# InterlinkLabs/e2e-tts

Hardware: AMD Instinct MI355X
Metric: audio samples/sec (22.05 kHz, batch-32 per GPU, FastSpeech2 + HiFi-GAN inference, ids on host -> int16 PCM on host) (higher is better)
Workload: dtype f32; 1 GPU; B=32/GPU fixed-length L=128 phonemes x 6 frames = T=768 frames (196608 samples, 8.92 s) per utterance; default model_config (6+6 FFT blocks H=384, HiFi-GAN V1), random-init weights; ids of tests/golden/bench_b32.npz (reference-pinned); global_batch=32, parallelism=utterance-sharded x1

## Files before the change

### e2e_tts_amd/csrc/attention.hip

```cpp
#include <math.h>

#include <algorithm>

#include "kernels.h"
#include "tuning.h"

namespace e2etts {

typedef float f32x16 __attribute__((ext_vector_type(16)));
typedef float f32x4v __attribute__((ext_vector_type(4)));
typedef unsigned u32x4v __attribute__((ext_vector_type(4)));

namespace {

__device__ __forceinline__ void lds_barrier() { asm volatile("s_waitcnt lgkmcnt(0)\n\ts_barrier" ::: "memory"); }

__device__ __forceinline__ void wave_lds_fence() {
  __builtin_amdgcn_fence(__ATOMIC_RELEASE, "wavefront");
  __builtin_amdgcn_wave_barrier();
  __builtin_amdgcn_fence(__ATOMIC_ACQUIRE, "wavefront");
}

constexpr int ATT_SEG_CHUNKS = 8;
__device__ __forceinline__ void seg_merge_ml(float& m, float& l, const float m_s, const float l_s, float& a, float& b) {
// ... 98 lines not shown
  }
}

template <int DT>
__device__ __forceinline__ void att_segment_close(f32x16 (&o)[DT], float& m_run, float& l_run, f32x16 (&ot)[DT], float& m_tot, float& l_tot,
                                                  const bool first) {
  if (first) {
#pragma unroll
    for (int d = 0; d < DT; ++d)
#pragma unroll
      for (int r = 0; r < 16; ++r) ot[d][r] = o[d][r];
    m_tot = m_run;
    l_tot = l_run;
  } else {
    float ma, mb;
    seg_merge_ml(m_tot, l_tot, m_run, l_run, ma, mb);
#pragma unroll
    for (int d = 0; d < DT; ++d)
#pragma unroll
      for (int r = 0; r < 16; ++r) ot[d][r] = seg_merge_o(ot[d][r], o[d][r], ma, mb);
  }
  att_clear(o);
  m_run = -INFINITY;
  l_run = 0.f;
}

template <int DT, int DK_BOUND>
__device__ __forceinline__ void att_store_rows(const f32x16 (&o)[DT], const float l, const bool valid, float* __restrict__ orow, const int lh) {
  const float inv = valid ? 1.0f / l : 0.f;
#pragma unroll
  for (int d = 0; d < DT; ++d)
#pragma unroll
    for (int g = 0; g < 4; ++g) {
      if (DK_BOUND % 32 == 0 || d * 32 + 8 * g + 4 * lh < DK_BOUND) {
        float4 v;
        v.x = valid ? o[d][4 * g + 0] * inv : 0.f;
        v.y = valid ? o[d][4 * g + 1] * inv : 0.f;
        v.z = valid ? o[d][4 * g + 2] * inv : 0.f;
        v.w = valid ? o[d][4 * g + 3] * inv : 0.f;
        *reinterpret_cast<float4*>(orow + d * 32 + 8 * g) = v;
      }
    }
}

template <int DK>
__global__ __launch_bounds__(256, 2) void attention_kernel(const float* __restrict__ qkv, float* __restrict__ out,
                                                        const int32_t* __restrict__ lens, int N, int H, float temperature, const RowMap rm) {
  constexpr int LDS_LD = DK + 4;
  constexpr int DT = DK / 32;
  constexpr int QQ = DK / 8;
  constexpr bool HALVES = DT % 2 == 0;
  __shared__ __attribute__((aligned(16))) float Ks[32 * LDS_LD];
  __shared__ __attribute__((aligned(16))) float Vs[32 * LDS_LD];

  const int tid = threadIdx.x, lane = tid & 63, wave = tid >> 6;
  const int li = lane & 31, lh = lane >> 5;
  ATT_BLOCK_OF_GRID(128)
  const int q0 = qblk * 128 + wave * 32;
  const int len = min(lens ? lens[b] : N, N);
  if (qblk * 128 >= len) {
    att_zero_tile<128, 256, DK>(out, b, qblk, head, N, H, tid);
    return;
  }
  const int ld = 3 * H;
  const float* base = qkv + (long long)b * N * ld;
  const float* qp = base + head * DK;
  const float* kp = base + H + head * DK;
  const float* vp = base + 2 * H + head * DK;

  float4 qf[QQ];
  att_load_q_f32(qf, qp + (long long)min(q0 + li, N - 1) * ld + lh * 4);

  f32x16 o[DT];
  att_clear(o);
  float m_run = -INFINITY, l_run = 0.f;
  f32x16 ot[DT];
  att_clear(ot);
  float m_tot = -INFINITY, l_tot = 0.f;

  const int nchunks = (len + 31) / 32;
  for (int sg0 = 0; sg0 < nchunks; sg0 += ATT_SEG_CHUNKS) {
  const int sg1 = min(nchunks, sg0 + ATT_SEG_CHUNKS);
  for (int kc = sg0; kc < sg1; ++kc) {
    __syncthreads();
    for (int i = tid; i < 32 * (DK / 4); i += 256) {
      const int r = i / (DK / 4), c = (i % (DK / 4)) * 4;
      const int key = kc * 32 + r;
      float4 kv = make_float4(0.f, 0.f, 0.f, 0.f), vv = kv;
      if (key < N) {
        kv = *reinterpret_cast<const float4*>(kp + (long long)key * ld + c);
        vv = *reinterpret_cast<const float4*>(vp + (long long)key * ld + c);
      }
      *reinterpret_cast<float4*>(Ks + r * LDS_LD + c) = kv;
      *reinterpret_cast<float4*>(Vs + r * LDS_LD + c) = vv;
    }
    __syncthreads();

    f32x16 s;
#pragma unroll
    for (int r = 0; r < 16; ++r) s[r] = 0.f;
    const float* ka = Ks + li * LDS_LD + lh * 4;
    if constexpr (HALVES) {
      f32x16 s1;
#pragma unroll
      for (int r = 0; r < 16; ++r) s1[r] = 0.f;
      att_qk_f32<0, QQ / 2>(s, ka, qf);
      att_qk_f32<QQ / 2, QQ>(s1, ka, qf);
#pragma unroll
      for (int r = 0; r < 16; ++r) s[r] = s[r] + s1[r];
    } else {
      att_qk_f32<0, QQ>(s, ka, qf);
    }
    float mx = -INFINITY;
#pragma unroll
    for (int r = 0; r < 16; ++r) {
      const int key = kc * 32 + (r & 3) + 8 * (r >> 2) + 4 * lh;
      float v = s[r] / temperature;
      v = key < len ? v : -INFINITY;
      s[r] = v;
      mx = fmaxf(mx, v);
    }
    mx = fmaxf(mx, __shfl_xor(mx, 32));
    const float m_new = fmaxf(m_run, mx);
    const float corr = expf(m_run - m_new);
    float psum = 0.f;
#pragma unroll
    for (int r = 0; r < 16; ++r) {
      const float pv = expf(s[r] - m_new);
      s[r] = pv;
      psum += pv;
    }
    psum += __shfl_xor(psum, 32);
    l_run = l_run * corr + psum;
    m_run = m_new;
    att_pv_f32<DT, LDS_LD>(o, s, corr, Vs + li, lh);
  }
    att_segment_close(o, m_run, l_run, ot, m_tot, l_tot, sg0 == 0);
  }

  const int q = q0 + li;
  if (q < N) att_store_rows<DT, DK>(ot, l_tot, q < len, out + ((long long)b * N + q) * H + head * DK + 4 * lh, lh);
}

template <int DK, int QT>
__global__ __launch_bounds__(QT * 128, 2) void attention_split_kernel(const float* __restrict__ qkv, float* __restrict__ out,
                                                                 const int32_t* __restrict__ lens, int N, int H, float temperature, const RowMap rm,
                                                                 float* __restrict__ ws_o, float* __restrict__ ws_ml, const int par_nseg) {
  constexpr int LDS_LD = DK + 4;
  constexpr int DH = DK / 2;
  constexpr int DTH = DH / 32;
  constexpr int QQH = DH / 8;
  static_assert(DK % 64 == 0, "the split form needs an even number of 32-wide head-dim tiles");
  constexpr int NF4 = 32 * (DK / 4);
  constexpr int NTH = QT * 128;
  constexpr int NLD = (NF4 + NTH - 1) / NTH;
  __shared__ __attribute__((aligned(16))) float Ks[32 * LDS_LD];
  __shared__ __attribute__((aligned(16))) float Vs[32 * LDS_LD];
  __shared__ __attribute__((aligned(16))) float Sx[QT * 2][16 * 64];

  const int tid = threadIdx.x, lane = tid & 63, wave = __builtin_amdgcn_readfirstlane(tid >> 6);
  const int li = lane & 31, lh = lane >> 5;
  const int qt = wave >> 1, part = wave & 1;
  ATT_BLOCK_OF_GRID(QT * 32)
  int seg_id = 0;
  if (par_nseg > 0) {
    seg_id = qblk % par_nseg;
    qblk /= par_nseg;
  }
  const int q0 = qblk * (QT * 32) + qt * 32;
  const int len = min(lens ? lens[b] : N, N);
  if (par_nseg > 0 && qblk * (QT * 32) >= len) return;
  if (qblk * (QT * 32) >= len) {
    att_zero_tile<QT * 32, NTH, DK>(out, b, qblk, head, N, H, tid);
    return;
  }
  const int ld = 3 * H;
  const float* base = qkv + (long long)b * N * ld;
  const float* qp = base + head * DK + part * DH;
  const float* kp = base + H + head * DK;
  const float* vp = base + 2 * H + head * DK;

  float4 qf[QQH];
  att_load_q_f32(qf, qp + (long long)min(q0 + li, N - 1) * ld + lh * 4);
  f32x16 o[DTH];
  att_clear(o);
  float m_run = -INFINITY, l_run = 0.f;

  float4 kreg[NLD], vreg[NLD];
  auto fetch = [&](int kc) __attribute__((always_inline)) {
#pragma unroll
    for (int i = 0; i < NLD; ++i) {
      const int idx = min(tid + i * NTH, NF4 - 1);
      const int r = idx / (DK / 4), c = (idx % (DK / 4)) * 4;
      const int key = min(kc * 32 + r, N - 1);
      kreg[i] = *reinterpret_cast<const float4*>(kp + (long long)key * ld + c);
      vreg[i] = *reinterpret_cast<const float4*>(vp + (long long)key * ld + c);
    }
  };
  auto stash = [&](int kc) __attribute__((always_inline)) {
#pragma unroll
    for (int i = 0; i < NLD; ++i) {
      const int idx = tid + i * NTH;
      if (idx < NF4) {
        const int r = idx / (DK / 4), c = (idx % (DK / 4)) * 4;
        const bool ok = kc * 32 + r < N;
        const float4 kv = make_float4(ok ? kreg[i].x : 0.f, ok ? kreg[i].y : 0.f, ok ? kreg[i].z : 0.f, ok ? kreg[i].w : 0.f);
        const float4 vv = make_float4(ok ? vreg[i].x : 0.f, ok ? vreg[i].y : 0.f, ok ? vreg[i].z : 0.f, ok ? vreg[i].w : 0.f);
        *reinterpret_cast<float4*>(Ks + r * LDS_LD + c) = kv;
        *reinterpret_cast<float4*>(Vs + r * LDS_LD + c) = vv;
      }
    }
  };

  const int nchunks = (len + 31) / 32;
  const int kc_begin = par_nseg > 0 ? seg_id * ATT_SEG_CHUNKS : 0;
  const int kc_end = par_nseg > 0 ? min(nchunks, (seg_id + 1) * ATT_SEG_CHUNKS) : nchunks;
  if (kc_begin >= kc_end) return;
  f32x16 ot[DTH];
  att_clear(ot);
  float m_tot = -INFINITY, l_tot = 0.f;
  fetch(kc_begin);
  for (int sg0 = kc_begin; sg0 < kc_end; sg0 += ATT_SEG_CHUNKS) {
  const int sg1 = min(kc_end, sg0 + ATT_SEG_CHUNKS);
  for (int kc = sg0; kc < sg1; ++kc) {
    lds_barrier();
    stash(kc);
    lds_barrier();
    if (kc + 1 < kc_end) fetch(kc + 1);

    f32x16 s;
#pragma unroll
    for (int r = 0; r < 16; ++r) s[r] = 0.f;
    att_qk_f32<0, QQH>(s, Ks + li * LDS_LD + part * DH + lh * 4, qf);
#pragma unroll
    for (int r = 0; r < 16; ++r) Sx[wave][r * 64 + lane] = s[r];
    lds_barrier();
    {
      const float* s0 = Sx[wave & ~1];
      const float* s1 = Sx[wave | 1];
#pragma unroll
      for (int r = 0; r < 16; ++r) s[r] = s0[r * 64 + lane] + s1[r * 64 + lane];
    }
    const float corr = att_softmax_step<true>(s, kc * 32, lh, len, temperature, m_run, l_run);
    att_pv_f32<DTH, LDS_LD>(o, s, corr, Vs + part * DH + li, lh);
  }
    if (par_nseg == 0) att_segment_close(o, m_run, l_run, ot, m_tot, l_tot, sg0 == kc_begin);
  }

  const int q = q0 + li;
  if (par_nseg > 0) {
    if (q < N) {
      const long long row = (((long long)b * (H / DK) + head) * par_nseg + seg_id) * N + q;
      float* orow = ws_o + row * DK + part * DH + 4 * lh;
#pragma unroll
      for (int d = 0; d < DTH; ++d)
#pragma unroll
        for (int g = 0; g < 4; ++g)
          *reinterpret_cast<float4*>(orow + d * 32 + 8 * g) = make_float4(o[d][4 * g], o[d][4 * g + 1], o[d][4 * g + 2], o[d][4 * g + 3]);
      if (part == 0 && lh == 0) *reinterpret_cast<float2*>(ws_ml + row * 2) = make_float2(m_run, l_run);
    }
    return;
  }
#pragma unroll
  for (int d = 0; d < DTH; ++d)
#pragma unroll
    for (int r = 0; r < 16; ++r) o[d][r] = ot[d][r];
  l_run = l_tot;
  if (q < N) att_store_rows<DTH, DH>(o, l_run, q < len, out + ((long long)b * N + q) * H + head * DK + part * DH + 4 * lh, lh);
}

__global__ void attention_combine_kernel(const float* __restrict__ ws_o, const float* __restrict__ ws_ml, float* __restrict__ out,
                                         const int32_t* __restrict__ lens, int N, int H, int DK, int par_nseg, long long total4) {
  const long long i = (long long)blockIdx.x * blockDim.x + threadIdx.x;
  if (i >= total4) return;
  const int d4 = DK / 4, nh = H / DK;
  const int c4 = (int)(i % d4);
  const int head = (int)((i / d4) % nh);
  const long long bq = i / ((long long)d4 * nh);
  const int q = (int)(bq % N), b = (int)(bq / N);
  const int len = min(lens ? lens[b] : N, N);
  float4 o = make_float4(0.f, 0.f, 0.f, 0.f);
  if (q < len) {
    const int nseg = ((len + 31) / 32 + ATT_SEG_CHUNKS - 1) / ATT_SEG_CHUNKS;
    float m = -INFINITY, l = 0.f;
    for (int sg = 0; sg < nseg; ++sg) {
      const long long row = (((long long)b * nh + head) * par_nseg + sg) * N + q;
      const float2 ml = *reinterpret_cast<const float2*>(ws_ml + row * 2);
      const float4 os = *reinterpret_cast<const float4*>(ws_o + row * DK + c4 * 4);
      if (sg == 0) {
        m = ml.x; l = ml.y; o = os;
      } else {
        float ma, mb;
        seg_merge_ml(m, l, ml.x, ml.y, ma, mb);
        o.x = seg_merge_o(o.x, os.x, ma, mb); o.y = seg_merge_o(o.y, os.y, ma, mb);
        o.z = seg_merge_o(o.z, os.z, ma, mb); o.w = seg_merge_o(o.w, os.w, ma, mb);
      }
    }
    const float inv = 1.0f / l;
    o.x *= inv; o.y *= inv; o.z *= inv; o.w *= inv;
  }
  *reinterpret_cast<float4*>(out + ((long long)b * N + q) * H + head * DK + c4 * 4) = o;
}

template <int DK>
__global__ __launch_bounds__(256, 2) void rel_attention_kernel(const float* __restrict__ qkv, const float* __restrict__ pos, int pos_rows,
                                                               const float* __restrict__ ub, const float* __restrict__ vb,
                                                               float* __restrict__ out, int N, int H, float temperature) {
  static_assert(DK % 8 == 0, "head dim must be a multiple of 8");
  constexpr int DT = (DK + 31) / 32;
  constexpr int LDS_LD = DT * 32 + 4;
  constexpr int QQ = DK / 8;
  constexpr int GLD = 68;
  constexpr int NPRE = QQ;
  __shared__ __attribute__((aligned(16))) float Ks[32 * LDS_LD];
  __shared__ __attribute__((aligned(16))) float Vs[32 * LDS_LD];
  __shared__ __attribute__((aligned(16))) float Gt[4][32 * GLD];

  const int tid = threadIdx.x, lane = tid & 63, wave = __builtin_amdgcn_readfirstlane(tid >> 6);
  const int li = lane & 31, lh = lane >> 5;
  const int b = blockIdx.z, head = blockIdx.y;
  const int i0 = blockIdx.x * 128 + wave * 32;
  const int ld = 3 * H;
  const float* base = qkv + (long long)b * N * ld;
  const float* qp = base + head * DK;
  const float* kp = base + H + head * DK;
  const float* vp = base + 2 * H + head * DK;
  const float* ph = pos + (long long)head * pos_rows * DK;
  float* const gt = Gt[wave];

  const int qi = min(i0 + li, N - 1);
  float4 qf[QQ], qx[QQ];
  auto load_qx = [&](const int row) __attribute__((always_inline)) {
    const float* qr = qp + (row * ld + lh * 4);
    const float* vr = vb + head * DK + lh * 4;
#pragma unroll
    for (int qq = 0; qq < QQ; ++qq) {
      const float4 a = *reinterpret_cast<const float4*>(qr + qq * 8), v4 = *reinterpret_cast<const float4*>(vr + qq * 8);
      qx[qq] = make_float4(a.x + v4.x, a.y + v4.y, a.z + v4.z, a.w + v4.w);
    }
  };
  {
    const float* qr = qp + (qi * ld + lh * 4);
    const float* ur = ub + head * DK + lh * 4;
#pragma unroll
    for (int qq = 0; qq < QQ; ++qq) {
      const float4 a = *reinterpret_cast<const float4*>(qr + qq * 8), u4 = *reinterpret_cast<const float4*>(ur + qq * 8);
      qf[qq] = make_float4(a.x + u4.x, a.y + u4.y, a.z + u4.z, a.w + u4.w);
    }
  }
  load_qx(qi);
  if (DK % 32) {
    for (int i = tid; i < 32 * (DT * 32 - DK); i += 256) {
      const int r = i / (DT * 32 - DK), c = DK + i % (DT * 32 - DK);
      Vs[r * LDS_LD + c] = 0.f;
    }
  }

  f32x16 o[DT];
  att_clear(o);
  float m_run = -INFINITY, l_run = 0.f;

  typedef f32x4v PRE_T;
  auto band_fetch = [&](PRE_T (&pre)[NPRE], const int row_start) __attribute__((always_inline)) {
    const int row = min(max(row_start + li, 0), pos_rows - 1);
    const float* pr = ph + (row * DK + lh * 4);
#pragma unroll
    for (int qq = 0; qq < QQ; ++qq) pre[qq] = *reinterpret_cast<const f32x4v*>(pr + qq * 8);
  };
  auto band_tile = [&](const PRE_T (&pre)[NPRE], const float4 (&x)[QQ]) __attribute__((always_inline)) -> f32x16 {
    f32x16 g;
#pragma unroll
    for (int r = 0; r < 16; ++r) g[r] = 0.f;
#pragma unroll
    for (int qq = 0; qq < QQ; ++qq) {
      g = __builtin_amdgcn_mfma_f32_32x32x2f32(pre[qq].x, x[qq].x, g, 0, 0, 0);
      g = __builtin_amdgcn_mfma_f32_32x32x2f32(pre[qq].y, x[qq].y, g, 0, 0, 0);
      g = __builtin_amdgcn_mfma_f32_32x32x2f32(pre[qq].z, x[qq].z, g, 0, 0, 0);
      g = __builtin_amdgcn_mfma_f32_32x32x2f32(pre[qq].w, x[qq].w, g, 0, 0, 0);
    }
    return g;
  };
  auto skew = [&](const f32x16& g0, const f32x16& g1, float (&term)[16], const bool diag) __attribute__((always_inline)) {
    wave_lds_fence();
#pragma unroll
    for (int q4 = 0; q4 < 4; ++q4) {
      const int t = 8 * q4 + 4 * lh;
      *reinterpret_cast<float4*>(gt + li * GLD + t) = make_float4(g0[4 * q4], g0[4 * q4 + 1], g0[4 * q4 + 2], g0[4 * q4 + 3]);
      *reinterpret_cast<float4*>(gt + li * GLD + 32 + t) = make_float4(g1[4 * q4], g1[4 * q4 + 1], g1[4 * q4 + 2], g1[4 * q4 + 3]);
    }
    wave_lds_fence();
#pragma unroll
    for (int r = 0; r < 16; ++r) {
      const int c = (r & 3) + 8 * (r >> 2) + 4 * lh;
      const float v = gt[li * GLD + (c - li + 31)];
      const bool keep = diag && c <= li, zero = diag && c == li + 1;
      term[r] = keep ? term[r] : (zero ? 0.f : v);
    }
  };
  auto new_tile_row = [&](const int j0, const bool upper) { return upper ? j0 - i0 - 1 : N + j0 - i0; };
  PRE_T pre[NPRE];
  f32x16 ghi;
#pragma unroll
  for (int r = 0; r < 16; ++r) ghi[r] = 0.f;

  const int nchunks = (N + 31) / 32;
  for (int kc = 0; kc < nchunks; ++kc) {
    const int j0 = kc * 32;
    __syncthreads();
    for (int i = tid; i < 32 * (DK / 4); i += 256) {
      const int r = i / (DK / 4), c = (i % (DK / 4)) * 4;
      const int key = j0 + r;
      float4 kv = make_float4(0.f, 0.f, 0.f, 0.f), vv = kv;
      if (key < N) {
        kv = *reinterpret_cast<const float4*>(kp + (key * ld + c));
        vv = *reinterpret_cast<const float4*>(vp + (key * ld + c));
      }
      *reinterpret_cast<float4*>(Ks + r * LDS_LD + c) = kv;
      *reinterpret_cast<float4*>(Vs + r * LDS_LD + c) = vv;
    }
    float pterm[16];
    if (j0 <= i0) {
      if (kc == 0) {
        band_fetch(pre, new_tile_row(j0, false) - 32);
        ghi = band_tile(pre, qx);
        band_fetch(pre, new_tile_row(j0, false));
      }
      const f32x16 g1 = band_tile(pre, qx);
      if (j0 < i0) band_fetch(pre, new_tile_row(j0 + 32, false));
      skew(ghi, g1, pterm, false);
      ghi = g1;
    }
    if (j0 >= i0) {
      if (j0 == i0) {
        load_qx(min(qi + 1, N - 1));
        band_fetch(pre, new_tile_row(j0, true) - 32);
        ghi = band_tile(pre, qx);
        band_fetch(pre, new_tile_row(j0, true));
      }
      const f32x16 g1 = band_tile(pre, qx);
      if (kc + 1 < nchunks) band_fetch(pre, new_tile_row(j0 + 32, true));
      skew(ghi, g1, pterm, j0 == i0);
      ghi = g1;
      if (j0 == i0 + 32 && li == 31 && lh == 0) pterm[0] = 0.f;
    }
    __syncthreads();

    f32x16 s;
#pragma unroll
    for (int r = 0; r < 16; ++r) s[r] = pterm[r];
    att_qk_f32<0, QQ>(s, Ks + li * LDS_LD + lh * 4, qf);
    const float corr = att_softmax_step<true>(s, j0, lh, N, temperature, m_run, l_run);
    att_pv_f32<DT, LDS_LD>(o, s, corr, Vs + li, lh);
  }

  const int q = i0 + li;
  if (q < N) att_store_rows<DT, DK>(o, l_run, true, out + ((long long)b * N + q) * H + head * DK + 4 * lh, lh);
}

typedef __bf16 bf16x8_t __attribute__((ext_vector_type(8)));
typedef __bf16 bf16x2_t __attribute__((ext_vector_type(2)));

__device__ __forceinline__ unsigned pk_bf16(float a, float b) {
  const bf16x2_t r = {(__bf16)a, (__bf16)b};
  return __builtin_bit_cast(unsigned, r);
}
__device__ __forceinline__ void split8(const float* v, bf16x8_t& hi, bf16x8_t& lo) {
  uint4 h, l;
  unsigned* hp = reinterpret_cast<unsigned*>(&h);
  unsigned* lp = reinterpret_cast<unsigned*>(&l);
#pragma unroll
  for (int i = 0; i < 4; ++i) {
    hp[i] = pk_bf16(v[2 * i], v[2 * i + 1]);
    const float h0 = __builtin_bit_cast(float, hp[i] << 16), h1 = __builtin_bit_cast(float, hp[i] & 0xffff0000u);
    lp[i] = pk_bf16(v[2 * i] - h0, v[2 * i + 1] - h1);
  }
  hi = __builtin_bit_cast(bf16x8_t, h);
  lo = __builtin_bit_cast(bf16x8_t, l);
}

constexpr int VS = 36;

template <int NS>
__device__ __forceinline__ void att_load_q_x3(bf16x8_t (&qh)[NS], bf16x8_t (&ql)[NS], const float* __restrict__ qr) {
#pragma unroll
  for (int s = 0; s < NS; ++s) {
    const float4 a = *reinterpret_cast<const float4*>(qr + s * 16), c = *reinterpret_cast<const float4*>(qr + s * 16 + 4);
    const float v[8] = {a.x, a.y, a.z, a.w, c.x, c.y, c.z, c.w};
    split8(v, qh[s], ql[s]);
  }
}

template <int DK, int VROWS>
__device__ __forceinline__ void att_stage_kv_x3(unsigned* Kh, unsigned* Vt, const int r, const int c4, const float4 kv, const float4 vv) {
  constexpr int KS = DK + 4;
  const unsigned k0 = pk_bf16(kv.x, kv.y), k1 = pk_bf16(kv.z, kv.w);
  const float kx = __builtin_bit_cast(float, k0 << 16), ky = __builtin_bit_cast(float, k0 & 0xffff0000u);
  const float kz = __builtin_bit_cast(float, k1 << 16), kw = __builtin_bit_cast(float, k1 & 0xffff0000u);
  *reinterpret_cast<uint2*>(Kh + r * KS + c4 * 2) = make_uint2(k0, k1);
  *reinterpret_cast<uint2*>(Kh + r * KS + DK / 2 + c4 * 2) = make_uint2(pk_bf16(kv.x - kx, kv.y - ky), pk_bf16(kv.z - kz, kv.w - kw));
  const int rr = (r & 3) + 4 * (r >> 3), h = (r >> 2) & 1;
  const int slot = 16 * (rr >> 3) + 8 * h + (rr & 7);
  unsigned short* vt = reinterpret_cast<unsigned short*>(Vt) + c4 * (VS * 2) + slot;
  const float vs[4] = {vv.x, vv.y, vv.z, vv.w};
#pragma unroll
  for (int e = 0; e < 4; ++e) {
    const __bf16 hb = (__bf16)vs[e];
    const __bf16 lb = (__bf16)(vs[e] - (float)hb);
    vt[e * VROWS * (VS * 2)] = __builtin_bit_cast(unsigned short, hb);
    vt[e * VROWS * (VS * 2) + 32] = __builtin_bit_cast(unsigned short, lb);
  }
}

template <int S0, int S1, int LO, int NS>
__device__ __forceinline__ void att_qk_x3(f32x16& s, const unsigned* ka, const bf16x8_t (&qh)[NS], const bf16x8_t (&ql)[NS]) {
#pragma unroll
  for (int ks = S0; ks < S1; ++ks) {
    const bf16x8_t ah = __builtin_bit_cast(bf16x8_t, *reinterpret_cast<const uint4*>(ka + ks * 8));
    const bf16x8_t al = __builtin_bit_cast(bf16x8_t, *reinterpret_cast<const uint4*>(ka + LO + ks * 8));
    s = __builtin_amdgcn_mfma_f32_32x32x16_bf16(al, qh[ks], s, 0, 0, 0);
    s = __builtin_amdgcn_mfma_f32_32x32x16_bf16(ah, ql[ks], s, 0, 0, 0);
    s = __builtin_amdgcn_mfma_f32_32x32x16_bf16(ah, qh[ks], s, 0, 0, 0);
  }
}

template <int DT, int PHYS>
__device__ __forceinline__ void att_pv_x3(f32x16 (&o)[DT], const f32x16& s, const float corr, const unsigned* Vt, const int t0, const int li, const int lh) {
  float pv[16];
#pragma unroll
  for (int r = 0; r < 16; ++r) pv[r] = s[r];
  bf16x8_t ph[2], pl[2];
  split8(pv, ph[0], pl[0]);
  split8(pv + 8, ph[1], pl[1]);
#pragma unroll
  for (int d = 0; d < DT; ++d) {
#pragma unroll
    for (int r = 0; r < 16; ++r) o[d][r] *= corr;
    const unsigned* va = Vt + ((li & 3) * PHYS + (t0 + d) * 8 + (li >> 2)) * VS + lh * 4;
#pragma unroll
    for (int s2 = 0; s2 < 2; ++s2) {
      const bf16x8_t ah = __builtin_bit_cast(bf16x8_t, *reinterpret_cast<const uint4*>(va + s2 * 8));
      const bf16x8_t al = __builtin_bit_cast(bf16x8_t, *reinterpret_cast<const uint4*>(va + 16 + s2 * 8));
      o[d] = __builtin_amdgcn_mfma_f32_32x32x16_bf16(al, ph[s2], o[d], 0, 0, 0);
      o[d] = __builtin_amdgcn_mfma_f32_32x32x16_bf16(ah, pl[s2], o[d], 0, 0, 0);
      o[d] = __builtin_amdgcn_mfma_f32_32x32x16_bf16(ah, ph[s2], o[d], 0, 0, 0);
    }
  }
}

template <int DK, int NW>
__global__ __launch_bounds__(NW * 64, 2) void attention_x3_kernel(const float* __restrict__ qkv, float* __restrict__ out,
                                                           const int32_t* __restrict__ lens, int N, int H, float temperature, const RowMap rm) {
  constexpr int KS = DK + 4;
  constexpr int DT = DK / 32;
  constexpr int NS = DK / 16;
  constexpr bool HALVES = DT % 2 == 0;
  static_assert(DK % 32 == 0, "head dim must be a multiple of 32");
  __shared__ __attribute__((aligned(16))) unsigned Kh[32 * KS];
  __shared__ __attribute__((aligned(16))) unsigned Vt[DK * VS];

  const int tid = threadIdx.x, lane = tid & 63, wave = tid >> 6;
  const int li = lane & 31, lh = lane >> 5;
  ATT_BLOCK_OF_GRID(NW * 32)
  const int q0 = qblk * (NW * 32) + wave * 32;
  const int len = min(lens ? lens[b] : N, N);
  if (qblk * (NW * 32) >= len) {
    att_zero_tile<NW * 32, NW * 64, DK>(out, b, qblk, head, N, H, tid);
    return;
  }
  const int ld = 3 * H;
  const float* base = qkv + (long long)b * N * ld;
  const float* qp = base + head * DK;
  const float* kp = base + H + head * DK;
  const float* vp = base + 2 * H + head * DK;

  bf16x8_t qh[NS], ql[NS];
  att_load_q_x3(qh, ql, qp + (long long)min(q0 + li, N - 1) * ld + lh * 8);

  f32x16 o[DT];
  att_clear(o);
  float m_run = -INFINITY, l_run = 0.f;
  const float inv_temp = 1.0f / temperature;

  const int nchunks = (len + 31) / 32;
  for (int kc = 0; kc < nchunks; ++kc) {
    __syncthreads();
    for (int i = tid; i < 32 * (DK / 4); i += NW * 64) {
      const int r = i / (DK / 4), c4 = i % (DK / 4);
      const int key = kc * 32 + r;
      float4 kv = make_float4(0.f, 0.f, 0.f, 0.f), vv = kv;
      if (key < N) {
        kv = *reinterpret_cast<const float4*>(kp + (key * ld + c4 * 4));
        vv = *reinterpret_cast<const float4*>(vp + (key * ld + c4 * 4));
      }
      att_stage_kv_x3<DK, DK / 4>(Kh, Vt, r, c4, kv, vv);
    }
    __syncthreads();

    f32x16 s;
#pragma unroll
    for (int r = 0; r < 16; ++r) s[r] = 0.f;
    const unsigned* ka = Kh + li * KS + lh * 4;
    if constexpr (HALVES) {
      f32x16 s1;
#pragma unroll
      for (int r = 0; r < 16; ++r) s1[r] = 0.f;
      att_qk_x3<0, NS / 2, DK / 2>(s, ka, qh, ql);
// ... 34 lines not shown
  const float* qp = base + head * DK;
  const float* kp = base + H + head * DK;
  const float* vp = base + 2 * H + head * DK;
  const unsigned* ph = posx + (long long)head * pos_rows * DK;
  float* const gt = Gt[wave];

  const int qi = min(i0 + li, N - 1);
  bf16x8_t fh[NS], fl[NS], xh[NS], xl[NS];
  auto load_frag = [&](const int row, const float* bias, bf16x8_t (&dh)[NS], bf16x8_t (&dl)[NS]) __attribute__((always_inline)) {
    const float* qr = qp + (row * ld + lh * 8);
    const float* br = bias + head * DK + lh * 8;
#pragma unroll
    for (int s = 0; s < NS; ++s) {
      const float4 a0 = *reinterpret_cast<const float4*>(qr + s * 16), a1 = *reinterpret_cast<const float4*>(qr + s * 16 + 4);
      const float4 b0 = *reinterpret_cast<const float4*>(br + s * 16), b1 = *reinterpret_cast<const float4*>(br + s * 16 + 4);
      const float t8[8] = {a0.x + b0.x, a0.y + b0.y, a0.z + b0.z, a0.w + b0.w, a1.x + b1.x, a1.y + b1.y, a1.z + b1.z, a1.w + b1.w};
      split8(t8, dh[s], dl[s]);
    }
  };
  load_frag(qi, ub, fh, fl);
  load_frag(qi, vb, xh, xl);

  f32x16 o[DTP];
  att_clear(o);
  float m_run = -INFINITY, l_run = 0.f;
  const float inv_temp = 1.0f / temperature;

  typedef u32x4v PRE_T;
  auto band_fetch = [&](PRE_T (&pre)[NPRE], const int row_start) __attribute__((always_inline)) {
    const int row = min(max(row_start + li, 0), pos_rows - 1);
    const unsigned* pr = ph + (row * DK + lh * 4);
#pragma unroll
    for (int ks = 0; ks < NS; ++ks) {
      pre[2 * ks] = *reinterpret_cast<const u32x4v*>(pr + ks * 8);
      pre[2 * ks + 1] = *reinterpret_cast<const u32x4v*>(pr + DK / 2 + ks * 8);
    }
  };
  auto band_tile = [&](const PRE_T (&pre)[NPRE]) __attribute__((always_inline)) -> f32x16 {
    f32x16 g;
#pragma unroll
    for (int r = 0; r < 16; ++r) g[r] = 0.f;
#pragma unroll
    for (int ks = 0; ks < NS; ++ks) {
      const bf16x8_t ah = __builtin_bit_cast(bf16x8_t, pre[2 * ks]);
      const bf16x8_t al = __builtin_bit_cast(bf16x8_t, pre[2 * ks + 1]);
      g = __builtin_amdgcn_mfma_f32_32x32x16_bf16(al, xh[ks], g, 0, 0, 0);
      g = __builtin_amdgcn_mfma_f32_32x32x16_bf16(ah, xl[ks], g, 0, 0, 0);
      g = __builtin_amdgcn_mfma_f32_32x32x16_bf16(ah, xh[ks], g, 0, 0, 0);
    }
    return g;
  };
  auto skew = [&](const f32x16& g0, const f32x16& g1, float (&term)[16], const bool diag) __attribute__((always_inline)) {
    wave_lds_fence();
#pragma unroll
    for (int q4 = 0; q4 < 4; ++q4) {
      const int t = 8 * q4 + 4 * lh;
      *reinterpret_cast<float4*>(gt + li * GLD + t) = make_float4(g0[4 * q4], g0[4 * q4 + 1], g0[4 * q4 + 2], g0[4 * q4 + 3]);
      *reinterpret_cast<float4*>(gt + li * GLD + 32 + t) = make_float4(g1[4 * q4], g1[4 * q4 + 1], g1[4 * q4 + 2], g1[4 * q4 + 3]);
    }
    wave_lds_fence();
#pragma unroll
    for (int r = 0; r < 16; ++r) {
      const int c = (r & 3) + 8 * (r >> 2) + 4 * lh;
      const float v = gt[li * GLD + (c - li + 31)];
      const bool keep = diag && c <= li, zero = diag && c == li + 1;
      term[r] = keep ? term[r] : (zero ? 0.f : v);
    }
  };
  auto new_tile_row = [&](const int j0, const bool upper) { return upper ? j0 - i0 - 1 : N + j0 - i0; };
  PRE_T pre[NPRE];
  f32x16 ghi;
#pragma unroll
  for (int r = 0; r < 16; ++r) ghi[r] = 0.f;

  const int nchunks = (N + 31) / 32;
  for (int kc = 0; kc < nchunks; ++kc) {
    const int j0 = kc * 32;
    __syncthreads();
    for (int i = tid; i < 32 * (DK / 4); i += 256) {
      const int r = i / (DK / 4), c4 = i % (DK / 4);
      const int key = j0 + r;
      float4 kv = make_float4(0.f, 0.f, 0.f, 0.f), vv = kv;
      if (key < N) {
        kv = *reinterpret_cast<const float4*>(kp + (key * ld + c4 * 4));
        vv = *reinterpret_cast<const float4*>(vp + (key * ld + c4 * 4));
      }
      att_stage_kv_x3<DK, 8 * DTP>(Kh, Vt, r, c4, kv, vv);
    }
    float pterm[16];
    if (j0 <= i0) {
      if (kc == 0) {
        band_fetch(pre, new_tile_row(j0, false) - 32);
        ghi = band_tile(pre);
        band_fetch(pre, new_tile_row(j0, false));
      }
      const f32x16 g1 = band_tile(pre);
      if (j0 < i0) band_fetch(pre, new_tile_row(j0 + 32, false));
      skew(ghi, g1, pterm, false);
      ghi = g1;
    }
    if (j0 >= i0) {
      if (j0 == i0) {
        load_frag(min(qi + 1, N - 1), vb, xh, xl);
        band_fetch(pre, new_tile_row(j0, true) - 32);
        ghi = band_tile(pre);
        band_fetch(pre, new_tile_row(j0, true));
      }
      const f32x16 g1 = band_tile(pre);
      if (kc + 1 < nchunks) band_fetch(pre, new_tile_row(j0 + 32, true));
      skew(ghi, g1, pterm, j0 == i0);
      ghi = g1;
      if (j0 == i0 + 32 && li == 31 && lh == 0) pterm[0] = 0.f;
    }
    __syncthreads();

    f32x16 s;
#pragma unroll
    for (int r = 0; r < 16; ++r) s[r] = pterm[r];
    const unsigned* ka = Kh + li * KS + lh * 4;
#pragma unroll
    for (int ks = 0; ks < NS; ++ks) {
      const bf16x8_t ah = __builtin_bit_cast(bf16x8_t, *reinterpret_cast<const uint4*>(ka + ks * 8));
      const bf16x8_t al = __builtin_bit_cast(bf16x8_t, *reinterpret_cast<const uint4*>(ka + DK / 2 + ks * 8));
      s = __builtin_amdgcn_mfma_f32_32x32x16_bf16(al, fh[ks], s, 0, 0, 0);
      s = __builtin_amdgcn_mfma_f32_32x32x16_bf16(ah, fl[ks], s, 0, 0, 0);
      s = __builtin_amdgcn_mfma_f32_32x32x16_bf16(ah, fh[ks], s, 0, 0, 0);
    }
    float mx = -INFINITY;
#pragma unroll
    for (int r = 0; r < 16; ++r) {
      const int key = j0 + (r & 3) + 8 * (r >> 2) + 4 * lh;
      float v = s[r] * inv_temp;
      v = key < N ? v : -INFINITY;
      s[r] = v;
      mx = fmaxf(mx, v);
    }
    mx = fmaxf(mx, __shfl_xor(mx, 32));
    const float m_new = fmaxf(m_run, mx);
    const float corr = __expf(m_run - m_new);
    float psum = 0.f;
    float pv[16];
#pragma unroll
    for (int r = 0; r < 16; ++r) {
      pv[r] = __expf(s[r] - m_new);
      psum += pv[r];
    }
    psum += __shfl_xor(psum, 32);
    l_run = l_run * corr + psum;
    m_run = m_new;
    bf16x8_t pfh[2], pfl[2];
    split8(pv, pfh[0], pfl[0]);
    split8(pv + 8, pfh[1], pfl[1]);
#pragma unroll
    for (int d = 0; d < DTP; ++d) {
#pragma unroll
      for (int r = 0; r < 16; ++r) o[d][r] *= corr;
      const unsigned* va = Vt + ((li & 3) * (8 * DTP) + d * 8 + (li >> 2)) * VS + lh * 4;
#pragma unroll
      for (int s2 = 0; s2 < 2; ++s2) {
        const bf16x8_t ah = __builtin_bit_cast(bf16x8_t, *reinterpret_cast<const uint4*>(va + s2 * 8));
        const bf16x8_t al = __builtin_bit_cast(bf16x8_t, *reinterpret_cast<const uint4*>(va + 16 + s2 * 8));
        o[d] = __builtin_amdgcn_mfma_f32_32x32x16_bf16(al, pfh[s2], o[d], 0, 0, 0);
        o[d] = __builtin_amdgcn_mfma_f32_32x32x16_bf16(ah, pfl[s2], o[d], 0, 0, 0);
        o[d] = __builtin_amdgcn_mfma_f32_32x32x16_bf16(ah, pfh[s2], o[d], 0, 0, 0);
      }
    }
  }

  const int q = i0 + li;
  if (q < N) att_store_rows<DTP, DK>(o, l_run, true, out + ((long long)b * N + q) * H + head * DK + 4 * lh, lh);
}

template <int DK, int QT>
__global__ __launch_bounds__(QT * 128, 2) void attention_x3_split_kernel(const float* __restrict__ qkv, float* __restrict__ out,
                                                                    const int32_t* __restrict__ lens, int N, int H, float temperature, const RowMap rm) {
  constexpr int KS = DK + 4;
  constexpr int DH = DK / 2, DTH = DH / 32, NSH = DH / 16;
  static_assert(DK % 64 == 0, "the split form needs an even number of 32-wide head-dim tiles");
  constexpr int NF4 = 32 * (DK / 4);
  constexpr int NTH = QT * 128;
  constexpr int NLD = (NF4 + NTH - 1) / NTH;
  __shared__ __attribute__((aligned(16))) unsigned Kh[32 * KS];
  __shared__ __attribute__((aligned(16))) unsigned Vt[DK * VS];
  __shared__ __attribute__((aligned(16))) float Sx[QT * 2][16 * 64];

  const int tid = threadIdx.x, lane = tid & 63, wave = __builtin_amdgcn_readfirstlane(tid >> 6);
  const int li = lane & 31, lh = lane >> 5;
  const int qt = wave >> 1, part = wave & 1;
  ATT_BLOCK_OF_GRID(QT * 32)
  const int q0 = qblk * (QT * 32) + qt * 32;
  const int len = min(lens ? lens[b] : N, N);
  if (qblk * (QT * 32) >= len) {
    att_zero_tile<QT * 32, NTH, DK>(out, b, qblk, head, N, H, tid);
    return;
  }
  const int ld = 3 * H;
  const float* base = qkv + (long long)b * N * ld;
  const float* qp = base + head * DK + part * DH;
  const float* kp = base + H + head * DK;
  const float* vp = base + 2 * H + head * DK;

  bf16x8_t qh[NSH], ql[NSH];
  att_load_q_x3(qh, ql, qp + (long long)min(q0 + li, N - 1) * ld + lh * 8);
  f32x16 o[DTH];
  att_clear(o);
  float m_run = -INFINITY, l_run = 0.f;
  const float inv_temp = 1.0f / temperature;

  float4 kreg[NLD], vreg[NLD];
  auto fetch = [&](int kc) __attribute__((always_inline)) {
#pragma unroll
    for (int i = 0; i < NLD; ++i) {
      const int idx = min(tid + i * NTH, NF4 - 1);
      const int r = idx / (DK / 4), c4 = idx % (DK / 4);
      const int key = min(kc * 32 + r, N - 1);
      kreg[i] = *reinterpret_cast<const float4*>(kp + (long long)key * ld + c4 * 4);
      vreg[i] = *reinterpret_cast<const float4*>(vp + (long long)key * ld + c4 * 4);
    }
  };
  auto stash = [&](int kc) __attribute__((always_inline)) {
#pragma unroll
    for (int i = 0; i < NLD; ++i) {
      const int idx = tid + i * NTH;
      if (idx < NF4) {
        const int r = idx / (DK / 4), c4 = idx % (DK / 4);
        const bool ok = kc * 32 + r < N;
        const float4 kv = make_float4(ok ? kreg[i].x : 0.f, ok ? kreg[i].y : 0.f, ok ? kreg[i].z : 0.f, ok ? kreg[i].w : 0.f);
        const float4 vv = make_float4(ok ? vreg[i].x : 0.f, ok ? vreg[i].y : 0.f, ok ? vreg[i].z : 0.f, ok ? vreg[i].w : 0.f);
        att_stage_kv_x3<DK, DK / 4>(Kh, Vt, r, c4, kv, vv);
      }
    }
  };

  const int nchunks = (len + 31) / 32;
  fetch(0);
  for (int kc = 0; kc < nchunks; ++kc) {
    lds_barrier();
    stash(kc);
    lds_barrier();
    if (kc + 1 < nchunks) fetch(kc + 1);

    f32x16 s;
#pragma unroll
    for (int r = 0; r < 16; ++r) s[r] = 0.f;
    att_qk_x3<0, NSH, DK / 2>(s, Kh + li * KS + part * (DH / 2) + lh * 4, qh, ql);
#pragma unroll
    for (int r = 0; r < 16; ++r) Sx[wave][r * 64 + lane] = s[r];
    lds_barrier();
    {
      const float* s0 = Sx[wave & ~1];
      const float* s1 = Sx[wave | 1];
#pragma unroll
      for (int r = 0; r < 16; ++r) s[r] = s0[r * 64 + lane] + s1[r * 64 + lane];
    }
    const float corr = att_softmax_step<false>(s, kc * 32, lh, len, inv_temp, m_run, l_run);
    att_pv_x3<DTH, DK / 4>(o, s, corr, Vt, part * DTH, li, lh);
  }

  const int q = q0 + li;
  if (q < N) att_store_rows<DTH, DH>(o, l_run, q < len, out + ((long long)b * N + q) * H + head * DK + part * DH + 4 * lh, lh);
}

}

const char* launch_rel_attention(const float* qkv, const float* pos, int pos_rows, const float* u, const float* v, float* out, int B, int N,
                                 int H, int n_head, hipStream_t s, const float* pos_x3) {
  if (!qkv || !pos || !u || !v || !out) return "rel_attention: null pointer";
  if (B <= 0 || N <= 0 || n_head <= 0 || H % n_head || pos_rows < N) return "rel_attention: bad dims (the position table must cover N rows)";
  if (B > 65535 || n_head > 65535) return "rel_attention: batch / heads exceed the grid limit";
  if ((long long)N * 3 * H >= (1LL << 31) || (long long)pos_rows * (H / n_head) >= (1LL << 31)) return "rel_attention: one utterance must stay below 2^31 elements (32-bit offsets)";
  if (((uintptr_t)qkv | (uintptr_t)pos | (uintptr_t)u | (uintptr_t)v | (uintptr_t)out) & 15) return "rel_attention: buffers must be 16-byte aligned";
  const int dk = H / n_head;
  const float temperature = sqrtf((float)H);
  dim3 grid((N + 127) / 128, n_head, B);
  if (pos_x3) {
    if ((uintptr_t)pos_x3 & 15) return "rel_attention: buffers must be 16-byte aligned";
    const unsigned* px = reinterpret_cast<const unsigned*>(pos_x3);
    switch (dk) {
      case 16: hipLaunchKernelGGL(rel_attention_x3_kernel<16>, grid, dim3(256), 0, s, qkv, px, pos_rows, u, v, out, N, H, temperature); break;
      case 32: hipLaunchKernelGGL(rel_attention_x3_kernel<32>, grid, dim3(256), 0, s, qkv, px, pos_rows, u, v, out, N, H, temperature); break;
      case 48: hipLaunchKernelGGL(rel_attention_x3_kernel<48>, grid, dim3(256), 0, s, qkv, px, pos_rows, u, v, out, N, H, temperature); break;
      case 64: hipLaunchKernelGGL(rel_attention_x3_kernel<64>, grid, dim3(256), 0, s, qkv, px, pos_rows, u, v, out, N, H, temperature); break;
      case 96: hipLaunchKernelGGL(rel_attention_x3_kernel<96>, grid, dim3(256), 0, s, qkv, px, pos_rows, u, v, out, N, H, temperature); break;
      default: return "rel_attention: the split-precision form needs a head dim of 16, 32, 48, 64 or 96";
    }
    return hipGetLastError() == hipSuccess ? nullptr : "rel_attention: launch failed";
  }
  switch (dk) {
    case 8: hipLaunchKernelGGL(rel_attention_kernel<8>, grid, dim3(256), 0, s, qkv, pos, pos_rows, u, v, out, N, H, temperature); break;
    case 16: hipLaunchKernelGGL(rel_attention_kernel<16>, grid, dim3(256), 0, s, qkv, pos, pos_rows, u, v, out, N, H, temperature); break;
    case 32: hipLaunchKernelGGL(rel_attention_kernel<32>, grid, dim3(256), 0, s, qkv, pos, pos_rows, u, v, out, N, H, temperature); break;
    case 48: hipLaunchKernelGGL(rel_attention_kernel<48>, grid, dim3(256), 0, s, qkv, pos, pos_rows, u, v, out, N, H, temperature); break;
    case 64: hipLaunchKernelGGL(rel_attention_kernel<64>, grid, dim3(256), 0, s, qkv, pos, pos_rows, u, v, out, N, H, temperature); break;
    case 96: hipLaunchKernelGGL(rel_attention_kernel<96>, grid, dim3(256), 0, s, qkv, pos, pos_rows, u, v, out, N, H, temperature); break;
    default: return "rel_attention: head dim must be one of 8, 16, 32, 48, 64, 96";
  }
  hipError_t err = hipGetLastError();
  return err == hipSuccess ? nullptr : hipGetErrorString(err);
}

long long attention_par_max_grid() {
  return 512;
}

size_t attention_workspace_bytes(int B, int N, int H, int n_head) {
  const long long nseg = ((N + 31) / 32 + ATT_SEG_CHUNKS - 1) / ATT_SEG_CHUNKS;
  return (size_t)((long long)B * n_head * nseg * N * (H / n_head + 2) * 4);
}

const char* launch_attention(const float* qkv, float* out, const int32_t* lens, int B, int N, int H, int n_head, int x3,
                             hipStream_t s, const int32_t* lens_host, float* ws, size_t ws_bytes) {
  if (!qkv || !out) return "attention: null pointer";
  if (B <= 0 || N <= 0 || n_head <= 0 || H % n_head) return "attention: bad dims";
  if (((uintptr_t)qkv | (uintptr_t)out) & 15) return "attention: buffers must be 16-byte aligned";
  const int dk = H / n_head;
  const float temperature = (float)sqrt((double)dk);
  dim3 grid((N + 127) / 128, n_head, B);
  const long long split_env = tuning().att_split_max;
  const long long split_max = split_env >= 0 ? split_env : (x3 ? 512 : (1LL << 62));
  dim3 gs((N + 63) / 64, n_head, B);
  RowMap rm;
  auto shape = [&](dim3 padded, int qrows) -> dim3 {
    rm.n = 0;
    if (!lens || !lens_host || B > ROWMAP_MAX) return padded;
    rm.n = B;
    rm.identity();
    std::stable_sort(rm.idx, rm.idx + B, [&](unsigned char x, unsigned char y) { return lens_host[x] > lens_host[y]; });
    rm.cum[0] = 0;
    for (int k = 0; k < B; ++k) rm.cum[k + 1] = rm.cum[k] + (std::min(std::max(lens_host[rm.idx[k]], 0), N) + qrows - 1) / qrows * n_head;
    return dim3((unsigned)std::max(rm.cum[B], 1));
  };
  const bool split = (dk == 64 || dk == 128 || dk == 192) && (long long)gs.x * gs.y * gs.z <= split_max;
  if (x3 && split) {
    const dim3 gc = shape(gs, 64);
    switch (dk) {
      case 64: hipLaunchKernelGGL((attention_x3_split_kernel<64, 2>), gc, dim3(256), 0, s, qkv, out, lens, N, H, temperature, rm); break;
      case 128: hipLaunchKernelGGL((attention_x3_split_kernel<128, 2>), gc, dim3(256), 0, s, qkv, out, lens, N, H, temperature, rm); break;
      default: hipLaunchKernelGGL((attention_x3_split_kernel<192, 2>), gc, dim3(256), 0, s, qkv, out, lens, N, H, temperature, rm); break;
    }
    return hipGetLastError() == hipSuccess ? nullptr : "attention: launch failed";
  }
  if (x3) {
    dim3 g8((N + 255) / 256, n_head, B);
    const dim3 gc = shape(g8, 256);
    switch (dk) {
      case 32: hipLaunchKernelGGL((attention_x3_kernel<32, 8>), gc, dim3(512), 0, s, qkv, out, lens, N, H, temperature, rm); break;
      case 64: hipLaunchKernelGGL((attention_x3_kernel<64, 8>), gc, dim3(512), 0, s, qkv, out, lens, N, H, temperature, rm); break;
      case 96: hipLaunchKernelGGL((attention_x3_kernel<96, 8>), gc, dim3(512), 0, s, qkv, out, lens, N, H, temperature, rm); break;
      case 128: hipLaunchKernelGGL((attention_x3_kernel<128, 8>), gc, dim3(512), 0, s, qkv, out, lens, N, H, temperature, rm); break;
      case 192: hipLaunchKernelGGL((attention_x3_kernel<192, 8>), gc, dim3(512), 0, s, qkv, out, lens, N, H, temperature, rm); break;
      default: return "attention: head dim must be one of 32, 64, 96, 128, 192";
    }
    return hipGetLastError() == hipSuccess ? nullptr : "attention: launch failed";
  }
  if (split) {
    dim3 gc = shape(gs, 64);
    const int nseg = ((N + 31) / 32 + ATT_SEG_CHUNKS - 1) / ATT_SEG_CHUNKS;
    int par_nseg = 0;
    float *ws_o = nullptr, *ws_ml = nullptr;
    if (tuning().att_par && rm.n == 0 && nseg >= 2 && ws && ws_bytes >= attention_workspace_bytes(B, N, H, n_head) && (((uintptr_t)ws) & 15) == 0 &&
        (long long)gs.x * gs.y * gs.z <= attention_par_max_grid() && (long long)gs.x * nseg < (1LL << 31)) {
      par_nseg = nseg;
      ws_o = ws;
      ws_ml = ws + (long long)B * n_head * nseg * N * dk;
      gc = dim3(gs.x * nseg, gs.y, gs.z);
    }
    switch (dk) {
      case 64: hipLaunchKernelGGL((attention_split_kernel<64, 2>), gc, dim3(256), 0, s, qkv, out, lens, N, H, temperature, rm, ws_o, ws_ml, par_nseg); break;
      case 128: hipLaunchKernelGGL((attention_split_kernel<128, 2>), gc, dim3(256), 0, s, qkv, out, lens, N, H, temperature, rm, ws_o, ws_ml, par_nseg); break;
      default: hipLaunchKernelGGL((attention_split_kernel<192, 2>), gc, dim3(256), 0, s, qkv, out, lens, N, H, temperature, rm, ws_o, ws_ml, par_nseg); break;
    }
    if (hipGetLastError() != hipSuccess) return "attention: launch failed";
    if (par_nseg > 0) {
      const long long total4 = (long long)B * N * (H / 4);
      hipLaunchKernelGGL(attention_combine_kernel, dim3((unsigned)((total4 + 255) / 256)), dim3(256), 0, s, ws_o, ws_ml, out, lens, N, H, dk, par_nseg, total4);
    }
    return hipGetLastError() == hipSuccess ? nullptr : "attention: launch failed";
  }
  const dim3 gc = shape(grid, 128);
  switch (dk) {
    case 32: hipLaunchKernelGGL(attention_kernel<32>, gc, dim3(256), 0, s, qkv, out, lens, N, H, temperature, rm); break;
    case 64: hipLaunchKernelGGL(attention_kernel<64>, gc, dim3(256), 0, s, qkv, out, lens, N, H, temperature, rm); break;
    case 96: hipLaunchKernelGGL(attention_kernel<96>, gc, dim3(256), 0, s, qkv, out, lens, N, H, temperature, rm); break;
    case 128: hipLaunchKernelGGL(attention_kernel<128>, gc, dim3(256), 0, s, qkv, out, lens, N, H, temperature, rm); break;
    case 192: hipLaunchKernelGGL(attention_kernel<192>, gc, dim3(256), 0, s, qkv, out, lens, N, H, temperature, rm); break;
    default: return "attention: head dim must be one of 32, 64, 96, 128, 192";
  }
  return hipGetLastError() == hipSuccess ? nullptr : "attention: launch failed";
}

}
```

### e2e_tts_amd/csrc/tuning.h

```cpp
#pragma once

namespace e2etts {

struct Tuning {
  int wg_per_cu = 24;
  bool frag64 = true;
  bool frag32 = true;
  bool rows = true;
  long long att_split_max = -1;
  bool att_par = true;
  bool dwglu = true;
  long long voc_conc_frames = -1;
  bool bconv = true;
  bool bpair = true;
  bool brb = true;
  bool voc_group = true;
  bool voc_defer_join = true;
};

const Tuning& tuning();

}
```

### e2e_tts_amd/csrc/tuning.hip

```cpp
#include "tuning.h"
#ifdef E2ETTS_TEST_HOOKS
#include <stdlib.h>
#endif

namespace e2etts {

const Tuning& tuning() {
  static const Tuning table = [] {
    Tuning t;
#ifdef E2ETTS_TEST_HOOKS
    auto num = [](const char* name, long long unset) { const char* v = getenv(name); return v ? atoll(v) : unset; };
    auto on = [&](const char* name) { return num(name, 1) != 0; };
    t.wg_per_cu = (int)num("E2ETTS_WG_PER_CU", t.wg_per_cu);
    t.frag64 = on("E2ETTS_FRAG64");
    t.frag32 = getenv("E2ETTS_NO_FRAG32") == nullptr;
    t.rows = on("E2ETTS_ROWS");
    t.bconv = on("E2ETTS_BCONV");
    t.voc_conc_frames = num("E2ETTS_VOC_CONC_FRAMES", -1);
    t.voc_group = on("E2ETTS_VOC_GROUP");
    t.voc_defer_join = on("E2ETTS_VOC_DEFER_JOIN");
    t.att_split_max = num("E2ETTS_ATT_SPLIT_MAX", -1);
    t.att_par = on("E2ETTS_ATT_PAR");
    t.dwglu = on("E2ETTS_DWGLU");
    t.bpair = on("E2ETTS_BPAIR");
    t.brb = on("E2ETTS_BRB");
#endif
    return t;
  }();
  return table;
}

}
```

Baseline: 48.91 million audio samples/s.

## Add full-sequence MFMA attention kernel with double-buffered K/V for large grids

```diff
diff --git a/e2e_tts_amd/csrc/attention.hip b/e2e_tts_amd/csrc/attention.hip
--- a/e2e_tts_amd/csrc/attention.hip
+++ b/e2e_tts_amd/csrc/attention.hip
@@ -424,6 +424,187 @@
   *reinterpret_cast<float4*>(out + ((long long)b * N + q) * H + head * DK + c4 * 4) = o;
 }
 
+typedef float f32x2v __attribute__((ext_vector_type(2)));
+
+template <int DK, int NW>
+__global__ __launch_bounds__(NW * 64) void attention_full_kernel(const float* __restrict__ qkv, float* __restrict__ out,
+                                                                 const int32_t* __restrict__ lens, int N, int H, float temperature,
+                                                                 const RowMap rm) {
+  constexpr int LDS_LD = DK + 4;
+  constexpr int DT = DK / 16;
+  constexpr int QQ = DK / 8;
+  constexpr int ROWS = NW * 16, NTH = NW * 64;
+  constexpr int NU = 32 * (DK / 8);
+  static_assert(DK % 64 == 0, "two half-head chains of whole channel groups");
+  static_assert(NU <= NTH, "one staging unit per thread");
+  __shared__ __attribute__((aligned(16))) float Ks[2][32 * LDS_LD];
+  __shared__ __attribute__((aligned(16))) float Vs[2][32 * LDS_LD];
+
+  const int tid = threadIdx.x, lane = tid & 63, wave = __builtin_amdgcn_readfirstlane(tid >> 6);
+  const int lj = lane & 15, g = lane >> 4, gh = g & 1, ge = g >> 1;
+  ATT_BLOCK_OF_GRID(ROWS)
+  const int q0 = qblk * ROWS + wave * 16;
+  const int len = min(lens ? lens[b] : N, N);
+  if (qblk * ROWS >= len) {
+    att_zero_tile<ROWS, NTH, DK>(out, b, qblk, head, N, H, tid);
+    return;
+  }
+  const int ld = 3 * H;
+  const float* base = qkv + (long long)b * N * ld;
+  const float* qp = base + head * DK;
+  const float* kp = base + H + head * DK;
+  const float* vp = base + 2 * H + head * DK;
+  const bool active = q0 < len;
+
+  float qf[QQ][2];
+  {
+    const float* qr = qp + (long long)min(q0 + lj, N - 1) * ld + (ge + 4 * gh);
+#pragma unroll
+    for (int qq = 0; qq < QQ; ++qq) {
+      qf[qq][0] = qr[qq * 8];
+      qf[qq][1] = qr[qq * 8 + 2];
+    }
+  }
+  f32x4v o[DT];
+#pragma unroll
+  for (int d = 0; d < DT; ++d) o[d] = f32x4v{0.f, 0.f, 0.f, 0.f};
+  float m_run = -INFINITY, l_run = 0.f;
+  float m_tot = -INFINITY, l_tot = 0.f;
+
+  const int sr = tid / (DK / 8), sc = (tid % (DK / 8)) * 8;
+  f32x4v kreg[2], vreg[2];
+  auto fetch = [&](int kc) __attribute__((always_inline)) {
+    if (tid < NU) {
+      const long long row = (long long)min(kc * 32 + sr, N - 1) * ld + sc;
+      kreg[0] = *reinterpret_cast<const f32x4v*>(kp + row);
+      kreg[1] = *reinterpret_cast<const f32x4v*>(kp + row + 4);
+      vreg[0] = *reinterpret_cast<const f32x4v*>(vp + row);
+      vreg[1] = *reinterpret_cast<const f32x4v*>(vp + row + 4);
+    }
+  };
+  auto stash = [&](int kc) __attribute__((always_inline)) {
+    if (tid < NU) {
+      const bool ok = kc * 32 + sr < N;
+      float* kd = Ks[kc & 1] + sr * LDS_LD + sc;
+      float* vd = Vs[kc & 1] + sr * LDS_LD + sc;
+      const f32x4v z = {0.f, 0.f, 0.f, 0.f};
+      const f32x4v ke = {kreg[0][0], kreg[0][2], kreg[1][0], kreg[1][2]}, ko = {kreg[0][1], kreg[0][3], kreg[1][1], kreg[1][3]};
+      *reinterpret_cast<f32x4v*>(kd) = ok ? ke : z;
+      *reinterpret_cast<f32x4v*>(kd + 4) = ok ? ko : z;
+      *reinterpret_cast<f32x4v*>(vd) = ok ? vreg[0] : z;
+      *reinterpret_cast<f32x4v*>(vd + 4) = ok ? vreg[1] : z;
+    }
+  };
+
+  const int krow = 8 * ((lj >> 1) & 1) + 2 * (lj & 1) + (lj >> 3) + 4 * ((lj >> 2) & 1);
+  const int koff = krow * LDS_LD + 2 * g;
+  const int voff = (ge + 4 * gh) * LDS_LD + lj;
+  float* const orow = out + ((long long)b * N + min(q0 + lj, N - 1)) * H + head * DK + 4 * g;
+  const bool store = q0 + lj < N;
+
+  const int nchunks = (len + 31) / 32;
+  fetch(0);
+  stash(0);
+  if (1 < nchunks) fetch(1);
+  lds_barrier();
+  for (int sg0 = 0; sg0 < nchunks; sg0 += ATT_SEG_CHUNKS) {
+    const int sg1 = min(nchunks, sg0 + ATT_SEG_CHUNKS);
+    for (int kc = sg0; kc < sg1; ++kc) {
+      if (active) {
+        const float* ka = Ks[kc & 1] + koff;
+        const float* va = Vs[kc & 1] + voff;
+        f32x4v sa[2][2];
+#pragma unroll
+        for (int t = 0; t < 2; ++t)
+#pragma unroll
+          for (int h = 0; h < 2; ++h) sa[t][h] = f32x4v{0.f, 0.f, 0.f, 0.f};
+#pragma unroll
+        for (int qq = 0; qq < QQ / 2; ++qq)
+#pragma unroll
+          for (int h = 0; h < 2; ++h)
+#pragma unroll
+            for (int t = 0; t < 2; ++t) {
+              const int qh = qq + h * (QQ / 2);
+              const f32x2v a = *reinterpret_cast<const f32x2v*>(ka + t * 16 * LDS_LD + qh * 8);
+              sa[t][h] = __builtin_amdgcn_mfma_f32_16x16x4f32(a[0], qf[qh][0], sa[t][h], 0, 0, 0);
+              sa[t][h] = __builtin_amdgcn_mfma_f32_16x16x4f32(a[1], qf[qh][1], sa[t][h], 0, 0, 0);
+            }
+        float p[8];
+        float mx = -INFINITY;
+#pragma unroll
+        for (int i = 0; i < 8; ++i) {
+          const int t = i >> 2, r = i & 3;
+          const int key = kc * 32 + 16 * t + 8 * (r >> 1) + 2 * (r & 1) + ge + 4 * gh;
+          float v = (sa[t][0][r] + sa[t][1][r]) / temperature;
+          v = key < len ? v : -INFINITY;
+          p[i] = v;
+          mx = fmaxf(mx, v);
+        }
+        mx = fmaxf(mx, __shfl_xor(mx, 32));
+        mx = fmaxf(mx, __shfl_xor(mx, 16));
+        const float m_new = fmaxf(m_run, mx);
+        const float corr = expf(m_run - m_new);
+        float psum = 0.f;
+#pragma unroll
+        for (int i = 0; i < 8; ++i) {
+          const float pv = expf(p[i] - m_new);
+          p[i] = pv;
+          const float other = __shfl_xor(pv, 32);
+          psum += ge ? other : pv;
+          psum += ge ? pv : other;
+        }
+        psum += __shfl_xor(psum, 16);
+        l_run = l_run * corr + psum;
+        m_run = m_new;
+#pragma unroll
+        for (int d = 0; d < DT; ++d) {
+#pragma unroll
+          for (int r = 0; r < 4; ++r) o[d][r] *= corr;
+#pragma unroll
+          for (int i = 0; i < 8; ++i) {
+            const float a = va[(8 * (i >> 1) + 2 * (i & 1)) * LDS_LD + d * 16];
+            o[d] = __builtin_amdgcn_mfma_f32_16x16x4f32(a, p[i], o[d], 0, 0, 0);
+          }
+        }
+      }
+      if (kc + 1 < nchunks) {
+        stash(kc + 1);
+        if (kc + 2 < nchunks) fetch(kc + 2);
+      }
+      lds_barrier();
+    }
+    const bool first = sg0 == 0, last = sg1 == nchunks;
+    float ma = 0.f, mb = 0.f;
+    if (first) {
+      m_tot = m_run;
+      l_tot = l_run;
+    } else {
+      seg_merge_ml(m_tot, l_tot, m_run, l_run, ma, mb);
+    }
+    if (store && (active || last)) {
+      const float inv = q0 + lj < len ? 1.0f / l_tot : 0.f;
+#pragma unroll
+      for (int d = 0; d < DT; ++d) {
+        f32x4v t = o[d];
+        if (!first && active) {
+          const f32x4v ot =*reinterpret_cast<const f32x4v*>(orow + d * 16);
+#pragma unroll
+          for (int r = 0; r < 4; ++r) t[r] = seg_merge_o(ot[r], o[d][r], ma, mb);
+        }
+        if (last) {
+#pragma unroll
+          for (int r = 0; r < 4; ++r) t[r] = q0 + lj < len ? t[r] * inv : 0.f;
+        }
+        *reinterpret_cast<f32x4v*>(orow + d * 16) = t;
+      }
+    }
+#pragma unroll
+    for (int d = 0; d < DT; ++d) o[d] = f32x4v{0.f, 0.f, 0.f, 0.f};
+    m_run = -INFINITY;
+    l_run = 0.f;
+  }
+}
+
 template <int DK>
 __global__ __launch_bounds__(256, 2) void rel_attention_kernel(const float* __restrict__ qkv, const float* __restrict__ pos, int pos_rows,
                                                                const float* __restrict__ ub, const float* __restrict__ vb,
@@ -1064,6 +1245,8 @@
 long long attention_par_max_grid() {
   return 512;
 }
+
+constexpr long long ATT_FULL_MIN_GRID = 513;
 
 size_t attention_workspace_bytes(int B, int N, int H, int n_head) {
   const long long nseg = ((N + 31) / 32 + ATT_SEG_CHUNKS - 1) / ATT_SEG_CHUNKS;
@@ -1115,6 +1298,16 @@
     }
     return hipGetLastError() == hipSuccess ? nullptr : "attention: launch failed";
   }
+  const long long full_env = tuning().att_full_min;
+  if (split && (long long)gs.x * gs.y * gs.z >= (full_env >= 0 ? full_env : ATT_FULL_MIN_GRID)) {
+    const dim3 gc = shape(dim3((N + 191) / 192, n_head, B), 192);
+    switch (dk) {
+      case 64: hipLaunchKernelGGL((attention_full_kernel<64, 12>), gc, dim3(768), 0, s, qkv, out, lens, N, H, temperature, rm); break;
+      case 128: hipLaunchKernelGGL((attention_full_kernel<128, 12>), gc, dim3(768), 0, s, qkv, out, lens, N, H, temperature, rm); break;
+      default: hipLaunchKernelGGL((attention_full_kernel<192, 12>), gc, dim3(768), 0, s, qkv, out, lens, N, H, temperature, rm); break;
+    }
+    return hipGetLastError() == hipSuccess ? nullptr : "attention: launch failed";
+  }
   if (split) {
     dim3 gc = shape(gs, 64);
     const int nseg = ((N + 31) / 32 + ATT_SEG_CHUNKS - 1) / ATT_SEG_CHUNKS;
diff --git a/e2e_tts_amd/csrc/tuning.h b/e2e_tts_amd/csrc/tuning.h
--- a/e2e_tts_amd/csrc/tuning.h
+++ b/e2e_tts_amd/csrc/tuning.h
@@ -8,6 +8,7 @@
   bool frag32 = true;
   bool rows = true;
   long long att_split_max = -1;
+  long long att_full_min = -1;
   bool att_par = true;
   bool dwglu = true;
   long long voc_conc_frames = -1;
diff --git a/e2e_tts_amd/csrc/tuning.hip b/e2e_tts_amd/csrc/tuning.hip
--- a/e2e_tts_amd/csrc/tuning.hip
+++ b/e2e_tts_amd/csrc/tuning.hip
@@ -1,6 +1,7 @@
 #include "tuning.h"
 #ifdef E2ETTS_TEST_HOOKS
 #include <stdlib.h>
+#include <string.h>
 #endif
 
 namespace e2etts {
@@ -10,6 +11,7 @@
     Tuning t;
 #ifdef E2ETTS_TEST_HOOKS
     auto num = [](const char* name, long long unset) { const char* v = getenv(name); return v ? atoll(v) : unset; };
+    auto field2 = [](const char* name, long long unset) { const char* v = getenv(name); v = v ? strchr(v, ':') : nullptr; return v ? atoll(v + 1) : unset; };
     auto on = [&](const char* name) { return num(name, 1) != 0; };
     t.wg_per_cu = (int)num("E2ETTS_WG_PER_CU", t.wg_per_cu);
     t.frag64 = on("E2ETTS_FRAG64");
@@ -20,6 +22,7 @@
     t.voc_group = on("E2ETTS_VOC_GROUP");
     t.voc_defer_join = on("E2ETTS_VOC_DEFER_JOIN");
     t.att_split_max = num("E2ETTS_ATT_SPLIT_MAX", -1);
+    t.att_full_min = field2("E2ETTS_ATT_SPLIT_MAX", -1);
     t.att_par = on("E2ETTS_ATT_PAR");
     t.dwglu = on("E2ETTS_DWGLU");
     t.bpair = on("E2ETTS_BPAIR");
```

New measurement: 49.01 million audio samples/s (median of 6 runs). About the same (+0.2%).
